# ducha-aiki/affnet

Measured on NVIDIA H100. Metric: Mpix/s end-to-end HesAffNet(+OriNet)+HardNet, higher is better.
Workload: dtype fp16 operands (fp16 residual planes: AffNet/OriNet weights+activations, HardNet layer 2-3 weights), fp32 accumulate; stencils fp32

## Files before the change

### affnet_b200/csrc/net_impl.cuh

```cuda
#pragma once
#include <cuda_fp16.h>

#include <vector>

#include "common.cuh"

#define AG_ENGINE_SIMT 0
#define AG_ENGINE_TC 1
#define AG_ENGINE_TC_EXACT 2
#define AG_ENGINE_TC2 4
#define AG_ENGINE_TC2_BF16 5
#define AG_ENGINE_TC_FAST 3

struct ag_net {
    int kind;
    int engine;
    float* d_w[6];
    float* d_b[6];
    float* d_w1;
    __half* d_wx[6];
    __half* d_all_x;
    __half* d_wx_bf[6];
    __half* d_headh_bf;
    __half* d_wh[6];
// ... 2 lines not shown
    float* d_head_b;
    float w_inv_scale[6];
    float head_inv_scale;
    float* d_all;
    __half* d_all_h;
};

#include "tc_conv.cuh"

namespace ag {
size_t tc_act_bytes(int kind);
int tc_nsplit(int kind, int layer);
int tc_split_w(int kind);
tc::FirstSrc tc_src_patches(const float* patches);
tc::FirstSrc tc_src_pyramid(const ag_pyramid_plan_t* p, const float* pyr, const float* lafs, const int* oct, const int* lvl, int cap);
int tc_hardnet_forward(const ag_net* net, const tc::FirstSrc& src, int n, int group, const int* count, void* bufA, void* bufB, void* headbuf,
                       float* out, cudaStream_t st);
int tc_trunk_orinet(const ag_net* net, const tc::FirstSrc& src, int n, int group, const int* count, void* bufA, void* bufB, void* feat,
                    cudaStream_t st);
int tc_trunk_affnet(const ag_net* net, const tc::FirstSrc& src, int n, int group, const int* count, void* bufA, void* bufB, void* feat,
                    cudaStream_t st);
int tc_headx_forward(const ag_net* net, const void* feat, int n, int group, const int* count, float* out, float* angle, cudaStream_t st, float* raw = nullptr);
size_t tc_headx_bytes(int n);
void tcx_pack_layer(const float* wf, int ci, int co, int stride, int nsplit, int sw, float scale, std::vector<__half>& out, int bf16 = 0);
int tcx_nsplit(int kind, int layer);
int tcx_split_w(int kind, int layer);
int tcx_stride(int layer);
size_t tcx_act_bytes(int n);
int tcx_trunk_affori(const ag_net* net, const tc::FirstSrc& src, int n, int group, const int* count, void* bufA, void* bufB, void* feat,
                     cudaStream_t st, int upto);
int tcx_trunk_hardnet(const ag_net* net, const tc::FirstSrc& src, int n, int group, const int* count, void* bufA, void* bufB, void* headbuf,
                      cudaStream_t st, int upto, int bf16 = 0);
int tc_hardnet_head(const ag_net* net, const void* headbuf, int n, int group, const int* count, float* out, cudaStream_t st, int bf16 = 0);
}
```

### affnet_b200/csrc/nets_simt.cu

```cuda
#include <math.h>

#include <vector>

#include <cuda_bf16.h>

#include "net_impl.cuh"

namespace ag {

constexpr float BN_EPS = 1e-5f;
constexpr int CNT = 256;

struct LayerCfg {
    int cin, cout, stride, hin;
};
static const LayerCfg kAffCfg[6] = {{1, 16, 1, 32}, {16, 16, 1, 32}, {16, 32, 2, 32}, {32, 32, 1, 16}, {32, 64, 2, 16}, {64, 64, 1, 8}};
static const LayerCfg kHardCfg[6] = {{1, 32, 1, 32}, {32, 32, 1, 32}, {32, 64, 2, 32}, {64, 64, 1, 16}, {64, 128, 2, 16}, {128, 128, 1, 8}};

}

namespace ag {

template <int CIN, int COUT, int HIN, int STRIDE, int CT, int CK, bool NORM>
__global__ void __launch_bounds__(CNT) conv3x3_kernel(const float* __restrict__ in, float* __restrict__ out,
// ... 337 lines not shown
    for (int l = 1; l < 6; l++) {
        const int ci = cfg[l].cin, co = cfg[l].cout, ns = tc_nsplit(kind, l), nt = co / ns, kc = ci / 8;
        const float* wf = packed.data() + w_off[l];
        w_scale[l] = pow2_scale(wf, (size_t)9 * ci * co);
        wh_off[l] = packed_h.size();
        packed_h.resize(packed_h.size() + (size_t)9 * ci * co * (1 + sw));
        __half* dst = packed_h.data() + wh_off[l];
        for (int sp = 0; sp < ns; sp++)
            for (int tap = 0; tap < 9; tap++)
                for (int g = 0; g < kc; g++)
                    for (int part = 0; part <= sw; part++)
                        for (int nn = 0; nn < nt; nn++)
                            for (int e = 0; e < 8; e++) {
                                const float v = w_scale[l] * wf[((size_t)tap * ci + g * 8 + e) * co + sp * nt + nn];
                                const __half hi = __float2half_rn(v);
                                const __half val = part == 0 ? hi : __float2half_rn(v - __half2float(hi));
                                dst[(((((size_t)sp * 9 + tap) * kc + g) * (1 + sw) + part) * nt + nn) * 8 + e] = val;
                            }
    }
    std::vector<__half> packed_x;
    size_t wx_off[6] = {0, 0, 0, 0, 0, 0};
    for (int l = 1; l < 6; l++) {
        wx_off[l] = packed_x.size();
        tcx_pack_layer(packed.data() + w_off[l], cfg[l].cin, cfg[l].cout, tcx_stride(l), tcx_nsplit(kind, l), tcx_split_w(kind, l), w_scale[l], packed_x);
        while (packed_x.size() % 8) packed_x.push_back(__float2half_rn(0.f));
    }
    std::vector<__half> packed_bf;
    size_t wbf_off[6] = {0, 0, 0, 0, 0, 0}, headbf_off = 0;
    if (kind == AG_NET_HARDNET) {
        for (int l = 1; l < 6; l++) {
            wbf_off[l] = packed_bf.size();
            tcx_pack_layer(packed.data() + w_off[l], cfg[l].cin, cfg[l].cout, tcx_stride(l), tcx_nsplit(kind, l), tcx_split_w(kind, l), w_scale[l], packed_bf, 1);
            while (packed_bf.size() % 8) packed_bf.push_back(__float2half_rn(0.f));
        }
        headbf_off = packed_bf.size();
        packed_bf.resize(packed_bf.size() + (size_t)8192 * 128);
        const float* hw = packed.data() + hw_off;
        for (int pix = 0; pix < 64; pix++)
            for (int cg = 0; cg < 16; cg++)
                for (int o = 0; o < 128; o++)
                    for (int e = 0; e < 8; e++) {
                        const __nv_bfloat16 bv = __float2bfloat16_rn(hw[((size_t)(cg * 8 + e) * 64 + pix) * 128 + o]);
                        memcpy(&packed_bf[headbf_off + (((size_t)(pix * 16 + cg)) * 128 + o) * 8 + e], &bv, 2);
                    }
    }
    size_t headh_off = 0;
    float head_scale = 1.0f;
    if (kind == AG_NET_HARDNET) {
        while (packed_h.size() % 8) packed_h.push_back(__float2half_rn(0.f));
        headh_off = packed_h.size();
        packed_h.resize(packed_h.size() + (size_t)8192 * 128);
        __half* dst = packed_h.data() + headh_off;
        const float* hw = packed.data() + hw_off;
        for (int pix = 0; pix < 64; pix++)
            for (int cg = 0; cg < 16; cg++)
// ... 266 lines not shown
```

### affnet_b200/csrc/nets_tcx.cu

```cuda
#include <stdlib.h>
#include <string.h>

#include <vector>

#include <cuda_bf16.h>

#include "net_impl.cuh"
#include "tcx_conv.cuh"
#include "tcx_first.cuh"

namespace ag {
namespace tcx {

static int num_sms() {
    static int n = 0;
    if (n == 0) {
        int dev = 0;
        cudaGetDevice(&dev);
        cudaDeviceGetAttribute(&n, cudaDevAttrMultiProcessorCount, dev);
        if (n <= 0) n = 132;
    }
    return n;
}

static int ensure_smem_attr(const void* func, int bytes, bool* configured, const char* what) {
    int dev = 0;
    cudaGetDevice(&dev);
    dev &= 63;
    if (configured[dev]) return AG_OK;
    int rc = check_cuda(cudaFuncSetAttribute(func, cudaFuncAttributeMaxDynamicSharedMemorySize, bytes), what);
    if (rc == AG_OK) configured[dev] = true;
    return rc;
}

template <int CIN, int COUT, int H, int STRIDE, int NSPLIT, int STAGES, int OUT, int SA, int SW, int OSA, int BF = 0, int MC = 0, int PPS = 0>
static int launch_conv(const void* in, void* out, const __half* w, const float* b, float inv_scale, int n, int group, const int* count, cudaStream_t st) {
    using Cfg = XCfg<CIN, COUT, H, STRIDE, NSPLIT, STAGES, OUT, SA, SW, OSA>;
    auto kern = tcx_conv_kernel<CIN, COUT, H, STRIDE, NSPLIT, STAGES, OUT, SA, SW, OSA, BF, MC, PPS>;
    static bool configured[64] = {};
    int rc = ensure_smem_attr((const void*)kern, (int)Cfg::SMEM, configured, "tcx_conv smem attr");
    if (rc != AG_OK) return rc;
    XArgs a;
    a.in = (const __half*)in; a.out = out; a.wpk = w; a.bias = b; a.inv_scale = inv_scale; a.n = n; a.group = group; a.count = count;
    const int units = Cfg::In::PAIR ? (n + 1) / 2 : n;
    int gx = num_sms() / NSPLIT;
    if (gx > units) gx = units;
    if (gx < 1) gx = 1;
    if (MC) {
        cudaLaunchConfig_t cfg;
        memset(&cfg, 0, sizeof(cfg));
        cfg.gridDim = dim3(gx, NSPLIT); cfg.blockDim = dim3(Cfg::THREADS); cfg.dynamicSmemBytes = Cfg::SMEM; cfg.stream = st;
        cudaLaunchAttribute attr[1];
        attr[0].id = cudaLaunchAttributeClusterDimension;
        attr[0].val.clusterDim.x = 1; attr[0].val.clusterDim.y = 2; attr[0].val.clusterDim.z = 1;
        cfg.attrs = attr; cfg.numAttrs = 1;
        rc = check_cuda(cudaLaunchKernelEx(&cfg, kern, a), "tcx_conv cluster launch");
        if (rc != AG_OK) return rc;
    } else
        kern<<<dim3(gx, NSPLIT), Cfg::THREADS, Cfg::SMEM, st>>>(a);
    AG_CHECK_LAUNCH("tcx_conv_kernel");
    return AG_OK;
// ... 24 lines not shown
    for (size_t i = (size_t)blockIdx.x * blockDim.x + threadIdx.x; i < total; i += (size_t)gridDim.x * blockDim.x) {
        const int x = (int)(i % H), y = (int)((i / H) % H), c = (int)((i / ((size_t)H * H)) % C), pi = (int)(i / ((size_t)H * H * C));
        const int slots = layout_slots(layout);
        const size_t unit_halfs = (size_t)(C / 8) * slots * 8 * (osa ? 2 : 1);
        const int unit = layout_pair(layout) ? (pi >> 1) : pi;
        const int slot = layout_slot(layout, y, x, pi & 1);
        const __half* ub = buf + (size_t)unit * unit_halfs;
        float v = __half2float(ub[((size_t)(c / 8) * slots + slot) * 8 + (c & 7)]);
        if (osa) v += __half2float(ub[((size_t)(C / 8 + c / 8) * slots + slot) * 8 + (c & 7)]);
        out[i] = v;
    }
}

}

static __half bf16_bits_as_half(float v) {
    const __nv_bfloat16 b = __float2bfloat16_rn(v);
    __half h;
    memcpy(&h, &b, 2);
    return h;
}
static float bf16_round(float v) { return __bfloat162float(__float2bfloat16_rn(v)); }

void tcx_pack_layer(const float* wf, int ci, int co, int stride, int nsplit, int sw, float scale, std::vector<__half>& out, int bf16) {
    const int nt = co / nsplit;
    auto put = [&](int dy, int dx, int cin, int c, int part) {
        const float v = scale * wf[((size_t)(dy * 3 + dx) * ci + cin) * co + c];
        if (bf16) {
            const float hi = bf16_round(v);
            out.push_back(bf16_bits_as_half(part == 0 ? hi : v - hi));
        } else {
            const __half hi = __float2half_rn(v);
            out.push_back(part == 0 ? hi : __float2half_rn(v - __half2float(hi)));
        }
    };
    for (int sp = 0; sp < nsplit; sp++)
        for (int dy = 0; dy < 3; dy++)
            for (int j = 0; j < ci / 16; j++) {
                if (stride == 1) {
                    for (int kg = 0; kg < 2; kg++)
                        for (int part = 0; part <= sw; part++)
                            for (int dx = 0; dx < 3; dx++)
                                for (int c = 0; c < nt; c++)
                                    for (int e = 0; e < 8; e++) put(dy, dx, (2 * j + kg) * 8 + e, sp * nt + c, part);
                } else {
                    for (int kg = 0; kg < 2; kg++)
                        for (int part = 0; part <= sw; part++)
                            for (int dx = 0; dx < 3; dx += 2)
                                for (int c = 0; c < nt; c++)
                                    for (int e = 0; e < 8; e++) put(dy, dx, (2 * j + kg) * 8 + e, sp * nt + c, part);
                    for (int kg = 0; kg < 2; kg++)
                        for (int part = 0; part <= sw; part++)
                            for (int c = 0; c < nt; c++)
                                for (int e = 0; e < 8; e++) put(dy, 1, (2 * j + kg) * 8 + e, sp * nt + c, part);
                }
            }
}

int tcx_nsplit(int kind, int layer) { return (kind == AG_NET_HARDNET && layer >= 4) ? 2 : 1; }
#ifndef AG_HARD_SW2
#define AG_HARD_SW2 1
#endif
#ifndef AG_HARD_SW3
#define AG_HARD_SW3 1
#endif
#ifndef AG_HARD_SW4
#define AG_HARD_SW4 0
#endif
int tcx_split_w(int kind, int layer) { return kind == AG_NET_HARDNET ? (layer == 1 ? AG_HARD_SW2 : layer == 2 ? AG_HARD_SW3 : layer == 3 ? AG_HARD_SW4 : 0) : 1; }
int tcx_stride(int layer) { return (layer == 2 || layer == 4) ? 2 : 1; }

size_t tcx_act_bytes(int n) { return (size_t)(n + 1) * 65536; }

#ifndef AG_HARD_MC5
#define AG_HARD_MC5 1
#endif
#ifndef AG_HARD_MC6
#define AG_HARD_MC6 0
#endif
int tcx_trunk_affori(const ag_net* net, const tc::FirstSrc& src0, int n, int group, const int* count, void* bufA, void* bufB, void* feat,
                     cudaStream_t st, int upto) {
    using namespace tcx;
    tc::FirstSrc src = src0;
    src.w1 = net->d_w1; src.b1 = net->d_b[0]; src.w1_inv = net->w_inv_scale[0]; src.w1_scale = 1.0f / net->w_inv_scale[0];
    int rc;
    if (upto <= 2) return launch_first<16, 16, 1, 1, 1>(bufB, net->d_wx[1], net->d_b[1], net->w_inv_scale[1], n, group, count, st, src);
    if ((rc = launch_first<16, 16, 1, 1, 1, 0, 1>(nullptr, net->d_wx[1], net->d_b[1], net->w_inv_scale[1], n, group, count, st, src,
                                                   bufA, net->d_wx[2], net->d_b[2], net->w_inv_scale[2]))) return rc;
    if (upto <= 3) return AG_OK;
    if ((rc = launch_conv<32, 32, 16, 1, 1, 4, L_S2_8P, 1, 1, 1>(bufA, bufB, net->d_wx[3], net->d_b[3], net->w_inv_scale[3], n, group, count, st))) return rc;
    if (upto <= 4) return AG_OK;
    if ((rc = launch_conv<32, 64, 16, 2, 1, 2, L_S1_8P, 1, 1, 1>(bufB, bufA, net->d_wx[4], net->d_b[4], net->w_inv_scale[4], n, group, count, st))) return rc;
    if (upto <= 5) return AG_OK;
    return launch_conv<64, 64, 8, 1, 1, 2, L_HEAD, 1, 1, 1, 0, 0, 1>(bufA, feat, net->d_wx[5], net->d_b[5], net->w_inv_scale[5], n, group, count, st);
}

template <int BF>
static int trunk_hardnet_t(const ag_net* net, const tc::FirstSrc& src0, int n, int group, const int* count, void* bufA, void* bufB, void* headbuf,
                           cudaStream_t st, int upto) {
    using namespace tcx;
    tc::FirstSrc src = src0;
    src.w1 = net->d_w1; src.b1 = net->d_b[0]; src.w1_inv = net->w_inv_scale[0]; src.w1_scale = 1.0f / net->w_inv_scale[0];
    __half* const* wx = BF ? net->d_wx_bf : net->d_wx;
    int rc;
    if ((rc = launch_first<32, 32, 0, AG_HARD_SW2, 0, BF>(bufB, wx[1], net->d_b[1], net->w_inv_scale[1], n, group, count, st, src))) return rc;
    if (upto <= 2) return AG_OK;
    if ((rc = launch_conv<32, 64, 32, 2, 1, 2, L_S1_16, 0, AG_HARD_SW3, 0, BF>(bufB, bufA, wx[2], net->d_b[2], net->w_inv_scale[2], n, group, count, st))) return rc;
    if (upto <= 3) return AG_OK;
    if ((rc = launch_conv<64, 64, 16, 1, 1, 2, L_S2_8P, 0, AG_HARD_SW4, 0, BF>(bufA, bufB, wx[3], net->d_b[3], net->w_inv_scale[3], n, group, count, st))) return rc;
    if (upto <= 4) return AG_OK;
    if ((rc = launch_conv<64, 128, 16, 2, 2, 2, L_S1_8P, 0, 0, 0, BF, AG_HARD_MC5, 1>(bufB, bufA, wx[4], net->d_b[4], net->w_inv_scale[4], n, group, count, st))) return rc;
    if (upto <= 5) return AG_OK;
    return launch_conv<128, 128, 8, 1, 2, 2, L_HEAD, 0, 0, 0, BF, AG_HARD_MC6, 1>(bufA, headbuf, wx[5], net->d_b[5], net->w_inv_scale[5], n, group, count, st);
}

int tcx_trunk_hardnet(const ag_net* net, const tc::FirstSrc& src0, int n, int group, const int* count, void* bufA, void* bufB, void* headbuf,
                      cudaStream_t st, int upto, int bf16) {
    return bf16 ? trunk_hardnet_t<1>(net, src0, n, group, count, bufA, bufB, headbuf, st, upto)
                : trunk_hardnet_t<0>(net, src0, n, group, count, bufA, bufB, headbuf, st, upto);
}

}

using namespace ag;

extern "C" {

int ag_debug_tcx_layer(const ag_net_t* net, const float* d_patches, int n, int upto, float* d_out, void* d_ws, size_t ws_bytes, void* stream) {
    AG_REQUIRE(net && d_patches && d_out && d_ws, "NULL argument");
    AG_REQUIRE(upto >= 2 && upto <= 5 && n >= 1, "layer out of range");
    const size_t act = align_up(tcx_act_bytes(n), 256);
    AG_REQUIRE(ws_bytes >= 2 * act, "workspace too small");
    cudaStream_t st = (cudaStream_t)stream;
    char* base = (char*)d_ws;
    const tc::FirstSrc src = tc_src_patches(d_patches);
    const bool hard = net->kind == AG_NET_HARDNET;
// ... 57 lines not shown
```

### affnet_b200/csrc/tcx_conv.cuh

```cuda
#pragma once
#include <cuda_bf16.h>

#include "tc_conv.cuh"

#ifndef AG_CONV_PINGPONG
#define AG_CONV_PINGPONG 1
#endif

namespace ag {
namespace tcx {

using namespace ag::tc;

constexpr int XORDER = 5;

enum { CT_TOTAL, CT_WAIT_FULL, CT_TURN, CT_ISSUE, CT_MMA_WAIT, CT_EPILOGUE, CT_WG_BAR, CT_WAIT_EMPTY, CT_OTHER, CT_STATES };
#ifdef AG_CONV_TIMELINE
constexpr int CT_CTAS = 4, CT_LAUNCHES = 16, CT_EVENTS = 2048;
__device__ unsigned long long g_conv_tl[CT_LAUNCHES][CT_CTAS][9][CT_STATES];
__device__ unsigned long long g_conv_ev[CT_LAUNCHES][2][CT_EVENTS][3];
__device__ int g_conv_tl_launch[CT_CTAS];
struct ConvTimeline {
    unsigned long long t[CT_STATES];
    long long start, mark;
    int slot, warp, n_ev;
    __device__ static void claim(int* s_slot) {
        if (threadIdx.x == 0)
            *s_slot = (blockIdx.y == 0 && blockIdx.x < CT_CTAS) ? min(atomicAdd(&g_conv_tl_launch[blockIdx.x], 1), CT_LAUNCHES) : CT_LAUNCHES;
    }
    __device__ void init(const int* s_slot) {
        for (int i = 0; i < CT_STATES; i++) t[i] = 0;
        slot = *s_slot; warp = threadIdx.x >> 5; n_ev = 0;
        start = mark = clock64();
    }
    __device__ void lap(int state) { const long long now = clock64(); t[state] += (unsigned long long)(now - mark); mark = now; }
    __device__ void event(int k) {
        if (blockIdx.x == 0 && slot < CT_LAUNCHES && (threadIdx.x & 127) == 0 && n_ev < CT_EVENTS) g_conv_ev[slot][warp >> 2][n_ev][k] = (unsigned long long)mark;
        if (k == 2) n_ev++;
    }
    __device__ void finish() {
        t[CT_TOTAL] = (unsigned long long)(clock64() - start);
        if ((threadIdx.x & 31) == 0 && slot < CT_LAUNCHES)
            for (int i = 0; i < CT_STATES; i++) g_conv_tl[slot][blockIdx.x][warp][i] = t[i];
    }
};
#else
struct ConvTimeline {
    __device__ static void claim(int*) {}
    __device__ void init(const int*) {}
    __device__ void lap(int) {}
    __device__ void event(int) {}
    __device__ void finish() {}
};
#endif

enum XLayout { L_S2_16 = 0, L_S1_16 = 1, L_S2_8P = 2, L_S1_8P = 3, L_HEAD = 4 };

__device__ __forceinline__ void bulk_g2s_mc(void* dst, const void* src, uint32_t bytes, uint64_t* bar, uint16_t mask) {
    asm volatile("cp.async.bulk.shared::cluster.global.mbarrier::complete_tx::bytes.multicast::cluster [%0], [%1], %2, [%3], %4;" ::"r"(smem_u32(dst)),
                 "l"(src), "r"(bytes), "r"(smem_u32(bar)), "h"(mask)
                 : "memory");
}
__device__ __forceinline__ void mbar_arrive_cluster(uint64_t* bar, uint32_t cta) {
    asm volatile("{\n .reg .b32 ra;\n mapa.shared::cluster.u32 ra, %0, %1;\n mbarrier.arrive.release.cta.shared::cluster.b64 _, [ra];\n}\n" ::"r"(smem_u32(bar)), "r"(cta)
                 : "memory");
}
__device__ __forceinline__ void cluster_sync() {
    asm volatile("barrier.cluster.arrive.release.aligned;\n barrier.cluster.wait.acquire.aligned;" ::: "memory");
}

template <int BF>
__device__ __forceinline__ uint32_t pack2(float a, float b) {
    if (BF) { const __nv_bfloat162 h = __floats2bfloat162_rn(a, b); return *reinterpret_cast<const uint32_t*>(&h); }
    const __half2 h = __floats2half2_rn(a, b);
    return *reinterpret_cast<const uint32_t*>(&h);
}
template <int BF>
__device__ __forceinline__ float2 unpack2(uint32_t u) {
    if (BF) return make_float2(__uint_as_float(u << 16), __uint_as_float(u & 0xFFFF0000u));
// ... 40 lines not shown
    static constexpr int PAIR = (HOUT == 8) ? 1 : 0;
    static constexpr int W = HOUT;
    static constexpr int RW = W * (1 + PAIR);
    static constexpr int TILES = HOUT * RW / 128;
    static constexpr int NPLANES = (STRIDE == 1) ? 1 : 4;
    static constexpr int DATA = HOUT * RW;
    static constexpr int PLANE = DATA + RW;
    static constexpr int SLOT_STAGE = NPLANES * PLANE;
    static constexpr int LAYOUT = (STRIDE == 2) ? (PAIR ? L_S2_8P : L_S2_16) : (PAIR ? L_S1_8P : L_S1_16);
    static_assert(HOUT == 8 || HOUT == 16 || HOUT == 32, "map sizes of the three nets");
    static_assert(!(STRIDE == 1 && H == 32), "the 32x32 stride-1 layer lives in tcx_first.cuh");
};

struct XArgs {
    const __half* in;
    void* out;
    const __half* wpk;
    const float* bias;
    float inv_scale;
    int n, group;
    const int* count;
};

template <int CIN, int COUT, int H, int STRIDE, int NSPLIT, int STAGES, int OUT, int SA, int SW, int OSA>
struct XCfg {
    using In = XIn<H, STRIDE>;
    static constexpr int CO = COUT, STRD = STRIDE, OUTL = OUT, SPLIT_A = SA, SPLIT_W = SW, SPLIT_O = OSA;
    static constexpr int KC = CIN / 8, NT = COUT / NSPLIT, HOUT = In::HOUT;
    static constexpr int G = KC * (1 + SA);
    static constexpr int GS = STAGES * In::SLOT_STAGE + (STRIDE == 1 ? In::RW : 0);
    static constexpr int ACCW = 3 * NT;
    static constexpr int BLOCKS = 2 * In::TILES;
    static constexpr uint32_t W_BYTES = 9u * CIN * NT * 2u * (1 + SW);
    static constexpr uint32_t IN_BYTES = (uint32_t)G * GS * 16u;
    static constexpr uint32_t HI_IN_BYTES = (uint32_t)KC * In::NPLANES * In::DATA * 16u;
    static constexpr uint32_t UNIT_IN_BYTES = HI_IN_BYTES * (1 + SA);
    static constexpr int THREADS = 288;
    static constexpr size_t SMEM = 1024 + (size_t)W_BYTES + IN_BYTES;
    static constexpr size_t HI_OUT_BYTES = (size_t)(COUT / 8) * layout_slots(OUT) * 16;
    static constexpr size_t UNIT_OUT_BYTES = (OUT == L_HEAD) ? 0 : HI_OUT_BYTES * (1 + OSA);
    static constexpr int NR1 = (1 + SW) * 3 * NT;
    static constexpr int NRO = (1 + SW) * 2 * NT, NRE = (1 + SW) * NT;
    static_assert(CIN % 16 == 0 && NT % 16 == 0 && ACCW <= 256, "wgmma shape");
    static_assert(In::W == 8 || In::W == 16, "a warp's 16 accumulator rows hold whole image rows");
    static_assert(SA <= 1 && SW <= 1 && OSA <= 1, "split-precision switches are 0 | 1");
    static_assert(2 * STAGES + 1 <= 60, "barrier area");
    static_assert(SMEM <= 232448, "shared memory budget");
    static_assert(GS < 16384, "leading-byte offset field");
    static_assert(OUT == L_HEAD || layout_pair(OUT) || !In::PAIR, "a pair layer writes pair layouts or the head operand");
};

__device__ __forceinline__ float frag_left_even(float v1, int lane) { return __shfl_sync(0xffffffffu, v1, (lane + 28) & 31); }
__device__ __forceinline__ float frag_right_odd(float v0, int lane) { return __shfl_sync(0xffffffffu, v0, (lane + 4) & 31); }

__device__ __forceinline__ bool xpatch_valid(const XArgs& a, int pi) { return pi < a.n && (a.count == nullptr || (pi % a.group) < a.count[pi / a.group]); }

template <class Cfg, int BF>
__device__ __forceinline__ void xconv_block_issue(float* d, uint32_t a_t, uint32_t w_base) {
    using In = typename Cfg::In;
    constexpr int KC = Cfg::KC, NT = Cfg::NT, GS = Cfg::GS, RW = In::RW, SA = Cfg::SPLIT_A, SW = Cfg::SPLIT_W;
    constexpr uint32_t LBO_A = ((uint32_t)GS) << 16;
    wgmma_fence();
    if (Cfg::STRD == 1) {
#pragma unroll
        for (int dy = 0; dy < 3; dy++) {
#pragma unroll
            for (int j = 0; j < KC / 2; j++) {
                const uint32_t ahi = ((a_t + (uint32_t)(dy * RW + 2 * j * GS)) & 0x3FFFu) | LBO_A;
                const uint32_t alo = ((a_t + (uint32_t)(dy * RW + (KC + 2 * j) * GS)) & 0x3FFFu) | LBO_A;
                const uint32_t blk = w_base + (uint32_t)((dy * (KC / 2) + j) * 2 * Cfg::NR1);
                const uint32_t bhi = (blk & 0x3FFFu) | ((uint32_t)Cfg::NR1 << 16), blo = ((blk + 3 * NT) & 0x3FFFu) | ((uint32_t)Cfg::NR1 << 16);
                Wgmma<3 * NT, BF>::mma(d, desc64(ahi), desc64(bhi), (dy | j) != 0);
                if (SW) Wgmma<3 * NT, BF>::mma(d, desc64(ahi), desc64(blo), 1);
                if (SA) Wgmma<3 * NT, BF>::mma(d, desc64(alo), desc64(bhi), 1);
            }
        }
    } else {
#pragma unroll
        for (int dy = 0; dy < 3; dy++) {
            constexpr int PL = In::PLANE;
            const int py = (dy == 1) ? 0 : 1, ro = (dy == 0) ? 0 : 1;
#pragma unroll
            for (int j = 0; j < KC / 2; j++) {
                const uint32_t blk = w_base + (uint32_t)((dy * (KC / 2) + j) * 2 * (Cfg::NRO + Cfg::NRE));
                const uint32_t bo_hi = (blk & 0x3FFFu) | ((uint32_t)Cfg::NRO << 16), bo_lo = ((blk + 2 * NT) & 0x3FFFu) | ((uint32_t)Cfg::NRO << 16);
                const uint32_t be = blk + 2 * Cfg::NRO;
                const uint32_t be_hi = (be & 0x3FFFu) | ((uint32_t)Cfg::NRE << 16), be_lo = ((be + NT) & 0x3FFFu) | ((uint32_t)Cfg::NRE << 16);
                const uint32_t ao = a_t + (uint32_t)((py * 2 + 1) * PL + ro * RW);
                const uint32_t ao_hi = ((ao + (uint32_t)(2 * j * GS)) & 0x3FFFu) | LBO_A, ao_lo = ((ao + (uint32_t)((KC + 2 * j) * GS)) & 0x3FFFu) | LBO_A;
                Wgmma<2 * NT, BF>::mma(d, desc64(ao_hi), desc64(bo_hi), (dy | j) != 0);
                if (SW) Wgmma<2 * NT, BF>::mma(d, desc64(ao_hi), desc64(bo_lo), 1);
                if (SA) Wgmma<2 * NT, BF>::mma(d, desc64(ao_lo), desc64(bo_hi), 1);
                const uint32_t ae = a_t + (uint32_t)((py * 2 + 0) * PL + ro * RW);
                const uint32_t ae_hi = ((ae + (uint32_t)(2 * j * GS)) & 0x3FFFu) | LBO_A, ae_lo = ((ae + (uint32_t)((KC + 2 * j) * GS)) & 0x3FFFu) | LBO_A;
                Wgmma<NT, BF>::mma(d + NT, desc64(ae_hi), desc64(be_hi), (dy | j) != 0);
                if (SW) Wgmma<NT, BF>::mma(d + NT, desc64(ae_hi), desc64(be_lo), 1);
                if (SA) Wgmma<NT, BF>::mma(d + NT, desc64(ae_lo), desc64(be_hi), 1);
            }
        }
    }
    wgmma_commit();
}
template <class Cfg, int BF>
__device__ __forceinline__ void xconv_block_epilogue(const float* d, const XArgs& a, const float* s_bias, int u, int b, int split, int wq, int lane) {
    using In = typename Cfg::In;
    constexpr int NT = Cfg::NT, HOUT = Cfg::HOUT, W = In::W, PAIR = In::PAIR, COUT = Cfg::CO, OUT = Cfg::OUTL, OSA = Cfg::SPLIT_O;
    unsigned char* obase[2];
    bool ok[2];
    size_t lo_off = 0;
    const int i = lane >> 2, xi = PAIR ? (i & 3) : i;
    const bool has_l0 = xi > 0, has_r1 = xi < W / 2 - 1;
    static_assert(W == 16 || PAIR, "neighbour-paired row groups: 16 pixels, or 8 of each patch of a pair");
#pragma unroll
    for (int h = 0; h < 2; h++) {
        const int y = b * 4 + wq, x = 2 * xi + h, pi = PAIR ? 2 * u + (i >> 2) : u;
        ok[h] = xpatch_valid(a, pi);
        if (OUT == L_HEAD) {
            obase[h] = reinterpret_cast<unsigned char*>(a.out) + (((size_t)(pi >> 7) * (HOUT * HOUT * COUT / 8) + (size_t)(y * HOUT + x) * (COUT / 8)) * 128 + (pi & 127)) * 16;
            lo_off = (size_t)((a.n + 127) >> 7) * (HOUT * HOUT * COUT / 8) * 128 * 16;
        } else {
            const int ou = layout_pair(OUT) ? (pi >> 1) : pi;
            obase[h] = reinterpret_cast<unsigned char*>(a.out) + (size_t)ou * Cfg::UNIT_OUT_BYTES + (size_t)layout_slot(OUT, y, x, pi & 1) * 16;
            lo_off = (size_t)(COUT / 8) * layout_slots(OUT) * 16;
        }
    }
#pragma unroll
    for (int j = 0; j < NT / 8; j++) {
        const int c = j * 8 + 2 * (lane & 3);
        float v[2][2];
#pragma unroll
        for (int e = 0; e < 2; e++) {
            const float c00 = d[4 * j + e], c01 = d[4 * j + 2 + e];
            const float c10 = d[4 * (j + NT / 8) + e], c11 = d[4 * (j + NT / 8) + 2 + e];
            const float c20 = d[4 * (j + 2 * NT / 8) + e], c21 = d[4 * (j + 2 * NT / 8) + 2 + e];
            const float l0 = frag_left_even(c01, lane);
            float acc0, acc1;
            if (Cfg::STRD == 1) {
                const float r1 = frag_right_odd(c20, lane);
                const float t0 = c21 + c10, t1 = has_r1 ? r1 + c11 : c11;
                acc0 = has_l0 ? l0 + t0 : t0;
                acc1 = c00 + t1;
            } else {
                const float t0 = c10 + c20, t1 = c11 + c21;
                acc0 = has_l0 ? l0 + t0 : t0;
                acc1 = c00 + t1;
            }
            v[0][e] = fmaxf(fmaf(acc0, a.inv_scale, s_bias[c + e]), 0.f);
            v[1][e] = fmaxf(fmaf(acc1, a.inv_scale, s_bias[c + e]), 0.f);
        }
        const int ch = split * NT + c;
        const size_t goff = ((OUT == L_HEAD) ? (size_t)(ch / 8) * 128 * 16 : (size_t)(ch / 8) * layout_slots(OUT) * 16) + (ch & 7) * 2;
#pragma unroll
        for (int h = 0; h < 2; h++) {
            if (!ok[h]) continue;
            uint32_t hi, lo;
            split_pack2<OSA, BF>(v[h][0], v[h][1], hi, lo);
            *reinterpret_cast<uint32_t*>(obase[h] + goff) = hi;
            if (OSA) *reinterpret_cast<uint32_t*>(obase[h] + lo_off + goff) = lo;
        }
    }
}

template <int CIN, int COUT, int H, int STRIDE, int NSPLIT, int STAGES, int OUT, int SA, int SW, int OSA, int BF = 0, int MC = 0, int PPS = 0>
__global__ void __launch_bounds__(288, 1) tcx_conv_kernel(const XArgs a) {
    static_assert(MC == 0 || NSPLIT == 2, "multicast pairs the two channel-split CTAs");
    using Cfg = XCfg<CIN, COUT, H, STRIDE, NSPLIT, STAGES, OUT, SA, SW, OSA>;
    using In = typename Cfg::In;
    constexpr int ACCW = Cfg::ACCW, BLOCKS = Cfg::BLOCKS, GS = Cfg::GS, RW = In::RW;
    constexpr int PAIR = In::PAIR;
    constexpr bool PP = AG_CONV_PINGPONG && PPS;
    extern __shared__ __align__(1024) unsigned char smem[];
    uint64_t* full = reinterpret_cast<uint64_t*>(smem);
    uint64_t* empty = full + STAGES;
    uint64_t* wbar = empty + STAGES;
    float* s_bias = reinterpret_cast<float*>(smem + 512);
    unsigned char* sW = smem + 1024;
    unsigned char* sIn = sW + Cfg::W_BYTES;

    const int warp = threadIdx.x >> 5, lane = threadIdx.x & 31;
    const int split = blockIdx.y;
    const int n_units = PAIR ? (a.n + 1) >> 1 : a.n;

    int* s_tl_slot = reinterpret_cast<int*>(smem + 496);

    if (threadIdx.x < Cfg::NT) s_bias[threadIdx.x] = a.bias[split * Cfg::NT + threadIdx.x];
    if (threadIdx.x == 0) {
        for (int s = 0; s < STAGES; s++) { mbar_init(&full[s], 1); mbar_init(&empty[s], (PP ? 8 : 2) * (1 + MC)); }
        mbar_init(wbar, 1);
        asm volatile("fence.mbarrier_init.release.cluster;" ::: "memory");
    }
    ConvTimeline::claim(s_tl_slot);
    for (int i = threadIdx.x; i < (int)(Cfg::IN_BYTES / 16); i += blockDim.x) reinterpret_cast<uint4*>(sIn)[i] = make_uint4(0, 0, 0, 0);
    asm volatile("fence.proxy.async.shared::cta;" ::: "memory");
    __syncthreads();
    if (MC) cluster_sync();
    ConvTimeline tl;
    tl.init(s_tl_slot);
    auto release = [&](uint64_t* e) {
        if (MC) { mbar_arrive_cluster(e, 0); mbar_arrive_cluster(e, 1); }
        else mbar_arrive(e);
    };

    auto uvalid = [&](int u) -> bool { return PAIR ? (xpatch_valid(a, 2 * u) || xpatch_valid(a, 2 * u + 1)) : xpatch_valid(a, u); };

    if (warp == 8) {
        if (lane == 0) {
            mbar_expect_tx(wbar, Cfg::W_BYTES);
            bulk_g2s(sW, reinterpret_cast<const unsigned char*>(a.wpk) + (size_t)split * Cfg::W_BYTES, Cfg::W_BYTES, wbar);
            int it = 0;
            for (int u = blockIdx.x; u < n_units; u += gridDim.x) {
// ... 14 lines not shown
                        else bulk_g2s(dst, srcp, In::DATA * 16u, &full[s]);
                    }
                it++;
            }
            tl.lap(CT_OTHER);
            if (MC) {
                for (int k = 0; k < STAGES && k < it; k++) { const int j = it - 1 - k; mbar_wait(&empty[j % STAGES], (j / STAGES) & 1); }
            }
            tl.lap(CT_WAIT_EMPTY);
        }
    } else if (warp < 8) {
        const int wg = warp >> 2, wq = warp & 3;
        mbar_wait(wbar, 0);
        const uint32_t w_base = smem_u32(sW) >> 4;
        const uint32_t in_base = smem_u32(sIn) >> 4;
        int it = 0;
        for (int u = blockIdx.x; u < n_units; u += gridDim.x) {
            if (!uvalid(u)) continue;
            const int s = it % STAGES;
            tl.lap(CT_OTHER);
            mbar_wait(&full[s], (it / STAGES) & 1);
            tl.lap(CT_WAIT_FULL);
            const uint32_t st_base = in_base + (uint32_t)(s * In::SLOT_STAGE);
#pragma unroll 1
            for (int b = wg; b < BLOCKS; b += 2) {
                float d[ACCW / 2];
                if (PP && (wg == 1 || it > 0 || b > 0)) bar_sync(XORDER + wg, 256);
                tl.lap(CT_TURN);
                tl.event(0);
                xconv_block_issue<Cfg, BF>(d, st_base + (uint32_t)(b * 64), w_base);
                if (PP) asm volatile("bar.arrive %0, 256;" ::"r"(XORDER + (wg ^ 1)) : "memory");
                tl.lap(CT_ISSUE);
                wgmma_wait<0>();
                wgmma_reg_fence<ACCW / 2>(d);
                tl.lap(CT_MMA_WAIT);
                tl.event(1);
                if (PP && b + 2 >= BLOCKS && lane == 0) release(&empty[s]);
                xconv_block_epilogue<Cfg, BF>(d, a, s_bias, u, b, split, wq, lane);
                tl.lap(CT_EPILOGUE);
                tl.event(2);
            }
            if (!PP) {
                bar_sync(3 + wg, 128);
                tl.lap(CT_WG_BAR);
                if ((threadIdx.x & 127) == 0) release(&empty[s]);
            }
            it++;
        }
        if (PP && wg == 0 && it > 0) bar_sync(XORDER, 256);
        tl.lap(CT_OTHER);
    }
    tl.finish();
    __syncthreads();
    if (MC) cluster_sync();
}

}
}
```

Measured before the change: 682.7.

## Add in-flight wgmma schedule overlapping epilogue with next channel group's MMAs

Adds an XS_INFLIGHT schedule for the AffNet/OriNet layers 3-4 conv kernels. Each block's output channels are split into groups of 32, the weights are repacked per group, and the kernel keeps two accumulator sets so the next group's wgmma is issued before the current group's epilogue runs. This aims to hide MMA latency behind the bias/ReLU/store epilogue, at the cost of more wgmma issues with a smaller N and a different weight packing layout. Layer 5 switches from the old PPS flag to an equivalent ping-pong enum.

Result: no change. 682.5 (median of 6 runs) (-0.0%).

```diff
diff --git a/affnet_b200/csrc/net_impl.cuh b/affnet_b200/csrc/net_impl.cuh
--- a/affnet_b200/csrc/net_impl.cuh
+++ b/affnet_b200/csrc/net_impl.cuh
@@ -48,8 +48,9 @@
                     cudaStream_t st);
 int tc_headx_forward(const ag_net* net, const void* feat, int n, int group, const int* count, float* out, float* angle, cudaStream_t st, float* raw = nullptr);
 size_t tc_headx_bytes(int n);
-void tcx_pack_layer(const float* wf, int ci, int co, int stride, int nsplit, int sw, float scale, std::vector<__half>& out, int bf16 = 0);
+void tcx_pack_layer(const float* wf, int ci, int co, int stride, int nsplit, int ng, int sw, float scale, std::vector<__half>& out, int bf16 = 0);
 int tcx_nsplit(int kind, int layer);
+int tcx_group(int kind, int layer, int co);
 int tcx_split_w(int kind, int layer);
 int tcx_stride(int layer);
 size_t tcx_act_bytes(int n);
diff --git a/affnet_b200/csrc/nets_simt.cu b/affnet_b200/csrc/nets_simt.cu
--- a/affnet_b200/csrc/nets_simt.cu
+++ b/affnet_b200/csrc/nets_simt.cu
@@ -383,7 +383,8 @@
     size_t wx_off[6] = {0, 0, 0, 0, 0, 0};
     for (int l = 1; l < 6; l++) {
         wx_off[l] = packed_x.size();
-        tcx_pack_layer(packed.data() + w_off[l], cfg[l].cin, cfg[l].cout, tcx_stride(l), tcx_nsplit(kind, l), tcx_split_w(kind, l), w_scale[l], packed_x);
+        tcx_pack_layer(packed.data() + w_off[l], cfg[l].cin, cfg[l].cout, tcx_stride(l), tcx_nsplit(kind, l), tcx_group(kind, l, cfg[l].cout),
+                       tcx_split_w(kind, l), w_scale[l], packed_x);
         while (packed_x.size() % 8) packed_x.push_back(__float2half_rn(0.f));
     }
     std::vector<__half> packed_bf;
@@ -391,7 +392,8 @@
     if (kind == AG_NET_HARDNET) {
         for (int l = 1; l < 6; l++) {
             wbf_off[l] = packed_bf.size();
-            tcx_pack_layer(packed.data() + w_off[l], cfg[l].cin, cfg[l].cout, tcx_stride(l), tcx_nsplit(kind, l), tcx_split_w(kind, l), w_scale[l], packed_bf, 1);
+            tcx_pack_layer(packed.data() + w_off[l], cfg[l].cin, cfg[l].cout, tcx_stride(l), tcx_nsplit(kind, l), tcx_group(kind, l, cfg[l].cout),
+                           tcx_split_w(kind, l), w_scale[l], packed_bf, 1);
             while (packed_bf.size() % 8) packed_bf.push_back(__float2half_rn(0.f));
         }
         headbf_off = packed_bf.size();
diff --git a/affnet_b200/csrc/nets_tcx.cu b/affnet_b200/csrc/nets_tcx.cu
--- a/affnet_b200/csrc/nets_tcx.cu
+++ b/affnet_b200/csrc/nets_tcx.cu
@@ -33,10 +33,10 @@
     return rc;
 }
 
-template <int CIN, int COUT, int H, int STRIDE, int NSPLIT, int STAGES, int OUT, int SA, int SW, int OSA, int BF = 0, int MC = 0, int PPS = 0>
+template <int CIN, int COUT, int H, int STRIDE, int NSPLIT, int STAGES, int OUT, int SA, int SW, int OSA, int BF, int MC, int SCHED>
 static int launch_conv(const void* in, void* out, const __half* w, const float* b, float inv_scale, int n, int group, const int* count, cudaStream_t st) {
     using Cfg = XCfg<CIN, COUT, H, STRIDE, NSPLIT, STAGES, OUT, SA, SW, OSA>;
-    auto kern = tcx_conv_kernel<CIN, COUT, H, STRIDE, NSPLIT, STAGES, OUT, SA, SW, OSA, BF, MC, PPS>;
+    auto kern = tcx_conv_kernel<CIN, COUT, H, STRIDE, NSPLIT, STAGES, OUT, SA, SW, OSA, BF, MC, SCHED>;
     static bool configured[64] = {};
     int rc = ensure_smem_attr((const void*)kern, (int)Cfg::SMEM, configured, "tcx_conv smem attr");
     if (rc != AG_OK) return rc;
@@ -107,8 +107,8 @@
 }
 static float bf16_round(float v) { return __bfloat162float(__float2bfloat16_rn(v)); }
 
-void tcx_pack_layer(const float* wf, int ci, int co, int stride, int nsplit, int sw, float scale, std::vector<__half>& out, int bf16) {
-    const int nt = co / nsplit;
+void tcx_pack_layer(const float* wf, int ci, int co, int stride, int nsplit, int ng, int sw, float scale, std::vector<__half>& out, int bf16) {
+    const int nt = co / nsplit, nh = nt / ng;
     auto put = [&](int dy, int dx, int cin, int c, int part) {
         const float v = scale * wf[((size_t)(dy * 3 + dx) * ci + cin) * co + c];
         if (bf16) {
@@ -125,24 +125,33 @@
                 if (stride == 1) {
                     for (int kg = 0; kg < 2; kg++)
                         for (int part = 0; part <= sw; part++)
-                            for (int dx = 0; dx < 3; dx++)
-                                for (int c = 0; c < nt; c++)
-                                    for (int e = 0; e < 8; e++) put(dy, dx, (2 * j + kg) * 8 + e, sp * nt + c, part);
+                            for (int hf = 0; hf < nh; hf++)
+                                for (int dx = 0; dx < 3; dx++)
+                                    for (int c = 0; c < ng; c++)
+                                        for (int e = 0; e < 8; e++) put(dy, dx, (2 * j + kg) * 8 + e, sp * nt + hf * ng + c, part);
                 } else {
                     for (int kg = 0; kg < 2; kg++)
                         for (int part = 0; part <= sw; part++)
-                            for (int dx = 0; dx < 3; dx += 2)
-                                for (int c = 0; c < nt; c++)
-                                    for (int e = 0; e < 8; e++) put(dy, dx, (2 * j + kg) * 8 + e, sp * nt + c, part);
+                            for (int hf = 0; hf < nh; hf++)
+                                for (int dx = 0; dx < 3; dx += 2)
+                                    for (int c = 0; c < ng; c++)
+                                        for (int e = 0; e < 8; e++) put(dy, dx, (2 * j + kg) * 8 + e, sp * nt + hf * ng + c, part);
                     for (int kg = 0; kg < 2; kg++)
                         for (int part = 0; part <= sw; part++)
-                            for (int c = 0; c < nt; c++)
-                                for (int e = 0; e < 8; e++) put(dy, 1, (2 * j + kg) * 8 + e, sp * nt + c, part);
+                            for (int hf = 0; hf < nh; hf++)
+                                for (int c = 0; c < ng; c++)
+                                    for (int e = 0; e < 8; e++) put(dy, 1, (2 * j + kg) * 8 + e, sp * nt + hf * ng + c, part);
                 }
             }
 }
 
 int tcx_nsplit(int kind, int layer) { return (kind == AG_NET_HARDNET && layer >= 4) ? 2 : 1; }
+
+constexpr int SCHED_AFFORI[6] = {tcx::XS_PLAIN, tcx::XS_PLAIN, tcx::XS_PLAIN, tcx::XS_INFLIGHT, tcx::XS_INFLIGHT, tcx::XS_PINGPONG};
+constexpr int SCHED_HARD[6] = {tcx::XS_PLAIN, tcx::XS_PLAIN, tcx::XS_PLAIN, tcx::XS_PLAIN, tcx::XS_PINGPONG, tcx::XS_PINGPONG};
+int tcx_group(int kind, int layer, int co) {
+    return tcx::xconv_group(kind == AG_NET_HARDNET ? SCHED_HARD[layer] : SCHED_AFFORI[layer], co / tcx_nsplit(kind, layer));
+}
 #ifndef AG_HARD_SW2
 #define AG_HARD_SW2 1
 #endif
@@ -173,11 +182,11 @@
     if ((rc = launch_first<16, 16, 1, 1, 1, 0, 1>(nullptr, net->d_wx[1], net->d_b[1], net->w_inv_scale[1], n, group, count, st, src,
                                                    bufA, net->d_wx[2], net->d_b[2], net->w_inv_scale[2]))) return rc;
     if (upto <= 3) return AG_OK;
-    if ((rc = launch_conv<32, 32, 16, 1, 1, 4, L_S2_8P, 1, 1, 1>(bufA, bufB, net->d_wx[3], net->d_b[3], net->w_inv_scale[3], n, group, count, st))) return rc;
+    if ((rc = launch_conv<32, 32, 16, 1, 1, 4, L_S2_8P, 1, 1, 1, 0, 0, SCHED_AFFORI[3]>(bufA, bufB, net->d_wx[3], net->d_b[3], net->w_inv_scale[3], n, group, count, st))) return rc;
     if (upto <= 4) return AG_OK;
-    if ((rc = launch_conv<32, 64, 16, 2, 1, 2, L_S1_8P, 1, 1, 1>(bufB, bufA, net->d_wx[4], net->d_b[4], net->w_inv_scale[4], n, group, count, st))) return rc;
+    if ((rc = launch_conv<32, 64, 16, 2, 1, 2, L_S1_8P, 1, 1, 1, 0, 0, SCHED_AFFORI[4]>(bufB, bufA, net->d_wx[4], net->d_b[4], net->w_inv_scale[4], n, group, count, st))) return rc;
     if (upto <= 5) return AG_OK;
-    return launch_conv<64, 64, 8, 1, 1, 2, L_HEAD, 1, 1, 1, 0, 0, 1>(bufA, feat, net->d_wx[5], net->d_b[5], net->w_inv_scale[5], n, group, count, st);
+    return launch_conv<64, 64, 8, 1, 1, 2, L_HEAD, 1, 1, 1, 0, 0, SCHED_AFFORI[5]>(bufA, feat, net->d_wx[5], net->d_b[5], net->w_inv_scale[5], n, group, count, st);
 }
 
 template <int BF>
@@ -190,13 +199,13 @@
     int rc;
     if ((rc = launch_first<32, 32, 0, AG_HARD_SW2, 0, BF>(bufB, wx[1], net->d_b[1], net->w_inv_scale[1], n, group, count, st, src))) return rc;
     if (upto <= 2) return AG_OK;
-    if ((rc = launch_conv<32, 64, 32, 2, 1, 2, L_S1_16, 0, AG_HARD_SW3, 0, BF>(bufB, bufA, wx[2], net->d_b[2], net->w_inv_scale[2], n, group, count, st))) return rc;
+    if ((rc = launch_conv<32, 64, 32, 2, 1, 2, L_S1_16, 0, AG_HARD_SW3, 0, BF, 0, SCHED_HARD[2]>(bufB, bufA, wx[2], net->d_b[2], net->w_inv_scale[2], n, group, count, st))) return rc;
     if (upto <= 3) return AG_OK;
-    if ((rc = launch_conv<64, 64, 16, 1, 1, 2, L_S2_8P, 0, AG_HARD_SW4, 0, BF>(bufA, bufB, wx[3], net->d_b[3], net->w_inv_scale[3], n, group, count, st))) return rc;
+    if ((rc = launch_conv<64, 64, 16, 1, 1, 2, L_S2_8P, 0, AG_HARD_SW4, 0, BF, 0, SCHED_HARD[3]>(bufA, bufB, wx[3], net->d_b[3], net->w_inv_scale[3], n, group, count, st))) return rc;
     if (upto <= 4) return AG_OK;
-    if ((rc = launch_conv<64, 128, 16, 2, 2, 2, L_S1_8P, 0, 0, 0, BF, AG_HARD_MC5, 1>(bufB, bufA, wx[4], net->d_b[4], net->w_inv_scale[4], n, group, count, st))) return rc;
+    if ((rc = launch_conv<64, 128, 16, 2, 2, 2, L_S1_8P, 0, 0, 0, BF, AG_HARD_MC5, SCHED_HARD[4]>(bufB, bufA, wx[4], net->d_b[4], net->w_inv_scale[4], n, group, count, st))) return rc;
     if (upto <= 5) return AG_OK;
-    return launch_conv<128, 128, 8, 1, 2, 2, L_HEAD, 0, 0, 0, BF, AG_HARD_MC6, 1>(bufA, headbuf, wx[5], net->d_b[5], net->w_inv_scale[5], n, group, count, st);
+    return launch_conv<128, 128, 8, 1, 2, 2, L_HEAD, 0, 0, 0, BF, AG_HARD_MC6, SCHED_HARD[5]>(bufA, headbuf, wx[5], net->d_b[5], net->w_inv_scale[5], n, group, count, st);
 }
 
 int tcx_trunk_hardnet(const ag_net* net, const tc::FirstSrc& src0, int n, int group, const int* count, void* bufA, void* bufB, void* headbuf,
diff --git a/affnet_b200/csrc/tcx_conv.cuh b/affnet_b200/csrc/tcx_conv.cuh
--- a/affnet_b200/csrc/tcx_conv.cuh
+++ b/affnet_b200/csrc/tcx_conv.cuh
@@ -34,8 +34,8 @@
         start = mark = clock64();
     }
     __device__ void lap(int state) { const long long now = clock64(); t[state] += (unsigned long long)(now - mark); mark = now; }
-    __device__ void event(int k) {
-        if (blockIdx.x == 0 && slot < CT_LAUNCHES && (threadIdx.x & 127) == 0 && n_ev < CT_EVENTS) g_conv_ev[slot][warp >> 2][n_ev][k] = (unsigned long long)mark;
+    __device__ void event(int k, int ahead = 0) {
+        if (blockIdx.x == 0 && slot < CT_LAUNCHES && (threadIdx.x & 127) == 0 && n_ev + ahead < CT_EVENTS) g_conv_ev[slot][warp >> 2][n_ev + ahead][k] = (unsigned long long)mark;
         if (k == 2) n_ev++;
     }
     __device__ void finish() {
@@ -49,12 +49,15 @@
     __device__ static void claim(int*) {}
     __device__ void init(const int*) {}
     __device__ void lap(int) {}
-    __device__ void event(int) {}
+    __device__ void event(int, int = 0) {}
     __device__ void finish() {}
 };
 #endif
 
 enum XLayout { L_S2_16 = 0, L_S1_16 = 1, L_S2_8P = 2, L_S1_8P = 3, L_HEAD = 4 };
+
+enum XSched { XS_PLAIN = 0, XS_PINGPONG = 1, XS_INFLIGHT = 2 };
+__host__ __device__ constexpr int xconv_group(int sched, int nt) { return (sched == XS_INFLIGHT && nt > 32) ? 32 : nt; }
 
 __device__ __forceinline__ void bulk_g2s_mc(void* dst, const void* src, uint32_t bytes, uint64_t* bar, uint16_t mask) {
     asm volatile("cp.async.bulk.shared::cluster.global.mbarrier::complete_tx::bytes.multicast::cluster [%0], [%1], %2, [%3], %4;" ::"r"(smem_u32(dst)),
@@ -141,14 +144,16 @@
     const int* count;
 };
 
-template <int CIN, int COUT, int H, int STRIDE, int NSPLIT, int STAGES, int OUT, int SA, int SW, int OSA>
+template <int CIN, int COUT, int H, int STRIDE, int NSPLIT, int STAGES, int OUT, int SA, int SW, int OSA, int NGRP = 0>
 struct XCfg {
     using In = XIn<H, STRIDE>;
     static constexpr int CO = COUT, STRD = STRIDE, OUTL = OUT, SPLIT_A = SA, SPLIT_W = SW, SPLIT_O = OSA;
     static constexpr int KC = CIN / 8, NT = COUT / NSPLIT, HOUT = In::HOUT;
+    static constexpr int NG = NGRP ? NGRP : NT, NH = NT / NG;
     static constexpr int G = KC * (1 + SA);
     static constexpr int GS = STAGES * In::SLOT_STAGE + (STRIDE == 1 ? In::RW : 0);
     static constexpr int ACCW = 3 * NT;
+    static constexpr int GACC = 3 * NG / 2;
     static constexpr int BLOCKS = 2 * In::TILES;
     static constexpr uint32_t W_BYTES = 9u * CIN * NT * 2u * (1 + SW);
     static constexpr uint32_t IN_BYTES = (uint32_t)G * GS * 16u;
@@ -161,6 +166,7 @@
     static constexpr int NR1 = (1 + SW) * 3 * NT;
     static constexpr int NRO = (1 + SW) * 2 * NT, NRE = (1 + SW) * NT;
     static_assert(CIN % 16 == 0 && NT % 16 == 0 && ACCW <= 256, "wgmma shape");
+    static_assert(NG % 16 == 0 && NT % NG == 0, "channel groups");
     static_assert(In::W == 8 || In::W == 16, "a warp's 16 accumulator rows hold whole image rows");
     static_assert(SA <= 1 && SW <= 1 && OSA <= 1, "split-precision switches are 0 | 1");
     static_assert(2 * STAGES + 1 <= 60, "barrier area");
@@ -175,9 +181,9 @@
 __device__ __forceinline__ bool xpatch_valid(const XArgs& a, int pi) { return pi < a.n && (a.count == nullptr || (pi % a.group) < a.count[pi / a.group]); }
 
 template <class Cfg, int BF>
-__device__ __forceinline__ void xconv_block_issue(float* d, uint32_t a_t, uint32_t w_base) {
+__device__ __forceinline__ void xconv_block_issue(float* d, uint32_t a_t, uint32_t w_base, int hf = 0) {
     using In = typename Cfg::In;
-    constexpr int KC = Cfg::KC, NT = Cfg::NT, GS = Cfg::GS, RW = In::RW, SA = Cfg::SPLIT_A, SW = Cfg::SPLIT_W;
+    constexpr int KC = Cfg::KC, NT = Cfg::NT, NG = Cfg::NG, GS = Cfg::GS, RW = In::RW, SA = Cfg::SPLIT_A, SW = Cfg::SPLIT_W;
     constexpr uint32_t LBO_A = ((uint32_t)GS) << 16;
     wgmma_fence();
     if (Cfg::STRD == 1) {
@@ -187,11 +193,11 @@
             for (int j = 0; j < KC / 2; j++) {
                 const uint32_t ahi = ((a_t + (uint32_t)(dy * RW + 2 * j * GS)) & 0x3FFFu) | LBO_A;
                 const uint32_t alo = ((a_t + (uint32_t)(dy * RW + (KC + 2 * j) * GS)) & 0x3FFFu) | LBO_A;
-                const uint32_t blk = w_base + (uint32_t)((dy * (KC / 2) + j) * 2 * Cfg::NR1);
+                const uint32_t blk = w_base + (uint32_t)((dy * (KC / 2) + j) * 2 * Cfg::NR1 + hf * 3 * NG);
                 const uint32_t bhi = (blk & 0x3FFFu) | ((uint32_t)Cfg::NR1 << 16), blo = ((blk + 3 * NT) & 0x3FFFu) | ((uint32_t)Cfg::NR1 << 16);
-                Wgmma<3 * NT, BF>::mma(d, desc64(ahi), desc64(bhi), (dy | j) != 0);
-                if (SW) Wgmma<3 * NT, BF>::mma(d, desc64(ahi), desc64(blo), 1);
-                if (SA) Wgmma<3 * NT, BF>::mma(d, desc64(alo), desc64(bhi), 1);
+                Wgmma<3 * NG, BF>::mma(d, desc64(ahi), desc64(bhi), (dy | j) != 0);
+                if (SW) Wgmma<3 * NG, BF>::mma(d, desc64(ahi), desc64(blo), 1);
+                if (SA) Wgmma<3 * NG, BF>::mma(d, desc64(alo), desc64(bhi), 1);
             }
         }
     } else {
@@ -202,28 +208,29 @@
 #pragma unroll
             for (int j = 0; j < KC / 2; j++) {
                 const uint32_t blk = w_base + (uint32_t)((dy * (KC / 2) + j) * 2 * (Cfg::NRO + Cfg::NRE));
-                const uint32_t bo_hi = (blk & 0x3FFFu) | ((uint32_t)Cfg::NRO << 16), bo_lo = ((blk + 2 * NT) & 0x3FFFu) | ((uint32_t)Cfg::NRO << 16);
-                const uint32_t be = blk + 2 * Cfg::NRO;
+                const uint32_t bo = blk + (uint32_t)(hf * 2 * NG), be = blk + (uint32_t)(2 * Cfg::NRO + hf * NG);
+                const uint32_t bo_hi = (bo & 0x3FFFu) | ((uint32_t)Cfg::NRO << 16), bo_lo = ((bo + 2 * NT) & 0x3FFFu) | ((uint32_t)Cfg::NRO << 16);
                 const uint32_t be_hi = (be & 0x3FFFu) | ((uint32_t)Cfg::NRE << 16), be_lo = ((be + NT) & 0x3FFFu) | ((uint32_t)Cfg::NRE << 16);
                 const uint32_t ao = a_t + (uint32_t)((py * 2 + 1) * PL + ro * RW);
                 const uint32_t ao_hi = ((ao + (uint32_t)(2 * j * GS)) & 0x3FFFu) | LBO_A, ao_lo = ((ao + (uint32_t)((KC + 2 * j) * GS)) & 0x3FFFu) | LBO_A;
-                Wgmma<2 * NT, BF>::mma(d, desc64(ao_hi), desc64(bo_hi), (dy | j) != 0);
-                if (SW) Wgmma<2 * NT, BF>::mma(d, desc64(ao_hi), desc64(bo_lo), 1);
-                if (SA) Wgmma<2 * NT, BF>::mma(d, desc64(ao_lo), desc64(bo_hi), 1);
+                Wgmma<2 * NG, BF>::mma(d, desc64(ao_hi), desc64(bo_hi), (dy | j) != 0);
+                if (SW) Wgmma<2 * NG, BF>::mma(d, desc64(ao_hi), desc64(bo_lo), 1);
+                if (SA) Wgmma<2 * NG, BF>::mma(d, desc64(ao_lo), desc64(bo_hi), 1);
                 const uint32_t ae = a_t + (uint32_t)((py * 2 + 0) * PL + ro * RW);
                 const uint32_t ae_hi = ((ae + (uint32_t)(2 * j * GS)) & 0x3FFFu) | LBO_A, ae_lo = ((ae + (uint32_t)((KC + 2 * j) * GS)) & 0x3FFFu) | LBO_A;
-                Wgmma<NT, BF>::mma(d + NT, desc64(ae_hi), desc64(be_hi), (dy | j) != 0);
-                if (SW) Wgmma<NT, BF>::mma(d + NT, desc64(ae_hi), desc64(be_lo), 1);
-                if (SA) Wgmma<NT, BF>::mma(d + NT, desc64(ae_lo), desc64(be_hi), 1);
+                Wgmma<NG, BF>::mma(d + NG, desc64(ae_hi), desc64(be_hi), (dy | j) != 0);
+                if (SW) Wgmma<NG, BF>::mma(d + NG, desc64(ae_hi), desc64(be_lo), 1);
+                if (SA) Wgmma<NG, BF>::mma(d + NG, desc64(ae_lo), desc64(be_hi), 1);
             }
         }
     }
     wgmma_commit();
 }
 template <class Cfg, int BF>
-__device__ __forceinline__ void xconv_block_epilogue(const float* d, const XArgs& a, const float* s_bias, int u, int b, int split, int wq, int lane) {
+__device__ __forceinline__ void xconv_block_epilogue(const float* d, const XArgs& a, const float* s_bias, int u, int b, int split, int wq, int lane,
+                                                     int hf = 0) {
     using In = typename Cfg::In;
-    constexpr int NT = Cfg::NT, HOUT = Cfg::HOUT, W = In::W, PAIR = In::PAIR, COUT = Cfg::CO, OUT = Cfg::OUTL, OSA = Cfg::SPLIT_O;
+    constexpr int NG = Cfg::NG, HOUT = Cfg::HOUT, W = In::W, PAIR = In::PAIR, COUT = Cfg::CO, OUT = Cfg::OUTL, OSA = Cfg::SPLIT_O;
     unsigned char* obase[2];
     bool ok[2];
     size_t lo_off = 0;
@@ -244,14 +251,14 @@
         }
     }
 #pragma unroll
-    for (int j = 0; j < NT / 8; j++) {
-        const int c = j * 8 + 2 * (lane & 3);
+    for (int j = 0; j < NG / 8; j++) {
+        const int c = hf * NG + j * 8 + 2 * (lane & 3);
         float v[2][2];
 #pragma unroll
         for (int e = 0; e < 2; e++) {
             const float c00 = d[4 * j + e], c01 = d[4 * j + 2 + e];
-            const float c10 = d[4 * (j + NT / 8) + e], c11 = d[4 * (j + NT / 8) + 2 + e];
-            const float c20 = d[4 * (j + 2 * NT / 8) + e], c21 = d[4 * (j + 2 * NT / 8) + 2 + e];
+            const float c10 = d[4 * (j + NG / 8) + e], c11 = d[4 * (j + NG / 8) + 2 + e];
+            const float c20 = d[4 * (j + 2 * NG / 8) + e], c21 = d[4 * (j + 2 * NG / 8) + 2 + e];
             const float l0 = frag_left_even(c01, lane);
             float acc0, acc1;
             if (Cfg::STRD == 1) {
@@ -267,7 +274,7 @@
             v[0][e] = fmaxf(fmaf(acc0, a.inv_scale, s_bias[c + e]), 0.f);
             v[1][e] = fmaxf(fmaf(acc1, a.inv_scale, s_bias[c + e]), 0.f);
         }
-        const int ch = split * NT + c;
+        const int ch = split * Cfg::NT + c;
         const size_t goff = ((OUT == L_HEAD) ? (size_t)(ch / 8) * 128 * 16 : (size_t)(ch / 8) * layout_slots(OUT) * 16) + (ch & 7) * 2;
 #pragma unroll
         for (int h = 0; h < 2; h++) {
@@ -280,14 +287,17 @@
     }
 }
 
-template <int CIN, int COUT, int H, int STRIDE, int NSPLIT, int STAGES, int OUT, int SA, int SW, int OSA, int BF = 0, int MC = 0, int PPS = 0>
+template <int CIN, int COUT, int H, int STRIDE, int NSPLIT, int STAGES, int OUT, int SA, int SW, int OSA, int BF = 0, int MC = 0, int SCHED = XS_PLAIN>
 __global__ void __launch_bounds__(288, 1) tcx_conv_kernel(const XArgs a) {
     static_assert(MC == 0 || NSPLIT == 2, "multicast pairs the two channel-split CTAs");
-    using Cfg = XCfg<CIN, COUT, H, STRIDE, NSPLIT, STAGES, OUT, SA, SW, OSA>;
+    using Cfg = XCfg<CIN, COUT, H, STRIDE, NSPLIT, STAGES, OUT, SA, SW, OSA, xconv_group(SCHED, COUT / NSPLIT)>;
     using In = typename Cfg::In;
     constexpr int ACCW = Cfg::ACCW, BLOCKS = Cfg::BLOCKS, GS = Cfg::GS, RW = In::RW;
     constexpr int PAIR = In::PAIR;
-    constexpr bool PP = AG_CONV_PINGPONG && PPS;
+    constexpr bool PP = AG_CONV_PINGPONG && SCHED == XS_PINGPONG;
+    constexpr bool IF = SCHED == XS_INFLIGHT;
+    constexpr int GROUPS = BLOCKS / 2 * Cfg::NH;
+    static_assert(!IF || GROUPS >= 2, "the in-flight schedule overlaps a group's epilogue with the next group's MMAs");
     extern __shared__ __align__(1024) unsigned char smem[];
     uint64_t* full = reinterpret_cast<uint64_t*>(smem);
     uint64_t* empty = full + STAGES;
@@ -304,7 +314,7 @@
 
     if (threadIdx.x < Cfg::NT) s_bias[threadIdx.x] = a.bias[split * Cfg::NT + threadIdx.x];
     if (threadIdx.x == 0) {
-        for (int s = 0; s < STAGES; s++) { mbar_init(&full[s], 1); mbar_init(&empty[s], (PP ? 8 : 2) * (1 + MC)); }
+        for (int s = 0; s < STAGES; s++) { mbar_init(&full[s], 1); mbar_init(&empty[s], (PP || IF ? 8 : 2) * (1 + MC)); }
         mbar_init(wbar, 1);
         asm volatile("fence.mbarrier_init.release.cluster;" ::: "memory");
     }
@@ -365,28 +375,61 @@
             mbar_wait(&full[s], (it / STAGES) & 1);
             tl.lap(CT_WAIT_FULL);
             const uint32_t st_base = in_base + (uint32_t)(s * In::SLOT_STAGE);
+            if constexpr (IF) {
+                constexpr int NH = Cfg::NH;
+                float d[2][Cfg::GACC];
+                auto issue = [&](float* dg, int k) {
+                    uint32_t at = st_base + (uint32_t)((wg + 2 * (k / NH)) * 64), wb = w_base;
+                    asm volatile("" : "+r"(at), "+r"(wb));
+                    xconv_block_issue<Cfg, BF>(dg, at, wb, k % NH);
+                };
+                tl.event(0);
+                issue(d[0], 0);
+                tl.lap(CT_ISSUE);
+#pragma unroll
+                for (int k = 0; k < GROUPS; k++) {
+                    if (k + 1 < GROUPS) {
+                        tl.event(0, 1);
+                        issue(d[(k + 1) & 1], k + 1);
+                        tl.lap(CT_ISSUE);
+                        wgmma_wait<1>();
+                    } else {
+                        wgmma_wait<0>();
+                    }
+                    wgmma_reg_fence<Cfg::GACC>(d[k & 1]);
+                    tl.lap(CT_MMA_WAIT);
+                    tl.event(1);
+                    if (k + 1 == GROUPS && lane == 0) release(&empty[s]);
+                    int ln = lane;
+                    asm volatile("" : "+r"(ln));
+                    xconv_block_epilogue<Cfg, BF>(d[k & 1], a, s_bias, u, wg + 2 * (k / NH), split, wq, ln, k % NH);
+                    tl.lap(CT_EPILOGUE);
+                    tl.event(2);
+                }
+            } else {
 #pragma unroll 1
-            for (int b = wg; b < BLOCKS; b += 2) {
-                float d[ACCW / 2];
-                if (PP && (wg == 1 || it > 0 || b > 0)) bar_sync(XORDER + wg, 256);
-                tl.lap(CT_TURN);
-                tl.event(0);
-                xconv_block_issue<Cfg, BF>(d, st_base + (uint32_t)(b * 64), w_base);
-                if (PP) asm volatile("bar.arrive %0, 256;" ::"r"(XORDER + (wg ^ 1)) : "memory");
-                tl.lap(CT_ISSUE);
-                wgmma_wait<0>();
-                wgmma_reg_fence<ACCW / 2>(d);
-                tl.lap(CT_MMA_WAIT);
-                tl.event(1);
-                if (PP && b + 2 >= BLOCKS && lane == 0) release(&empty[s]);
-                xconv_block_epilogue<Cfg, BF>(d, a, s_bias, u, b, split, wq, lane);
-                tl.lap(CT_EPILOGUE);
-                tl.event(2);
-            }
-            if (!PP) {
-                bar_sync(3 + wg, 128);
-                tl.lap(CT_WG_BAR);
-                if ((threadIdx.x & 127) == 0) release(&empty[s]);
+                for (int b = wg; b < BLOCKS; b += 2) {
+                    float d[ACCW / 2];
+                    if (PP && (wg == 1 || it > 0 || b > 0)) bar_sync(XORDER + wg, 256);
+                    tl.lap(CT_TURN);
+                    tl.event(0);
+                    xconv_block_issue<Cfg, BF>(d, st_base + (uint32_t)(b * 64), w_base);
+                    if (PP) asm volatile("bar.arrive %0, 256;" ::"r"(XORDER + (wg ^ 1)) : "memory");
+                    tl.lap(CT_ISSUE);
+                    wgmma_wait<0>();
+                    wgmma_reg_fence<ACCW / 2>(d);
+                    tl.lap(CT_MMA_WAIT);
+                    tl.event(1);
+                    if (PP && b + 2 >= BLOCKS && lane == 0) release(&empty[s]);
+                    xconv_block_epilogue<Cfg, BF>(d, a, s_bias, u, b, split, wq, lane);
+                    tl.lap(CT_EPILOGUE);
+                    tl.event(2);
+                }
+                if (!PP) {
+                    bar_sync(3 + wg, 128);
+                    tl.lap(CT_WG_BAR);
+                    if ((threadIdx.x & 127) == 0) release(&empty[s]);
+                }
             }
             it++;
         }
```
